# Ascend-Research/HeadPoseEstimation-WHENet

Hardware: AMD Instinct MI355X
Metric: head crops/sec (224x224) (higher is better)
Workload: dtype f16

## Files before the change

### __graft_entry__.py

```python
from __future__ import annotations

import os
import subprocess
import sys
from concurrent.futures import ThreadPoolExecutor

ROOT = os.path.dirname(os.path.abspath(__file__))
PKG = os.path.join(ROOT, "headposeestimation-whenet_amd")
CSRC = os.path.join(PKG, "csrc")
LIBDIR = os.path.join(PKG, "lib")
OBJDIR = os.path.join(PKG, "build")
LIB = os.path.join(LIBDIR, "libwhenet_hip.so")

SOURCES = ["stem.hip", "stemdw.hip", "dw.hip", "se.hip", "pw.hip", "head.hip", "head7.hip", "front.hip", "front2.hip", "front2s.hip", "front7.hip", "mb7.hip", "frame.hip", "headplan.hip", "letterbox.hip", "yolo.hip", "dconv.hip", "convert.hip", "yuv.hip", "ingest.hip", "overlay.hip", "jpeg.hip", "jpeg_dec.hip", "jpeg_dec_seg.hip",
           "snapshot.cpp", "engine.cpp", "engine_post.cpp", "engine_ops.cpp", "detector.cpp", "capi.cpp"]
HEADERS = ["common.h", "spec.h", "snapshot.h", "kernels.h", "device_math.h", "engine.h", "engine_internal.h", "stamps.h", "se_device.h", "overlay_host.h", "jpeg_host.h", "jpeg_dec_host.h", "jpeg_dec_seg_host.h", "front_tuned_f16.inc", "front_tuned_f32.inc", "front2_tuned.inc", "front2s_tuned.inc",
           os.path.join("..", "..", "include", "whenet_hip.h")]
EXTRA_FLAGS = {"front2.hip": ["-mllvm", "-amdgpu-mfma-vgpr-form"], "front2s.hip": ["-mllvm", "-amdgpu-mfma-vgpr-form"], "front7.hip": ["-mllvm", "-amdgpu-mfma-vgpr-form"],
               "mb7.hip": ["-mllvm", "-amdgpu-mfma-vgpr-form"],
               "overlay.hip": ["-ffp-contract=off"]}
CXXFLAGS = ["--offload-arch=gfx950", "-mcode-object-version=5", "-O3", "-std=c++17", "-fPIC", "-Wall",
            "-Wno-unused-function", "-fvisibility=hidden"]


def _hipcc() -> str:
    for cand in (os.environ.get("HIPCC"), "/opt/rocm/bin/hipcc", "hipcc"):
        if cand and (os.path.isabs(cand) and os.path.exists(cand) or not os.path.isabs(cand)):
            return cand
    raise RuntimeError("hipcc not found")


def _stale(target: str, deps) -> bool:
    if not os.path.exists(target):
        return True
    t = os.path.getmtime(target)
    return any(os.path.getmtime(d) > t for d in deps if os.path.exists(d))


def build(force: bool = False, verbose: bool = False) -> None:
    os.makedirs(LIBDIR, exist_ok=True)
    os.makedirs(OBJDIR, exist_ok=True)
    hipcc = _hipcc()
    hdrs = [os.path.join(CSRC, h) for h in HEADERS]

    def compile_one(src: str) -> str:
        s = os.path.join(CSRC, src)
        o = os.path.join(OBJDIR, src.replace(".", "_") + ".o")
        if force or _stale(o, [s] + hdrs):
            cmd = [hipcc] + CXXFLAGS + EXTRA_FLAGS.get(src, []) + ["-c", s, "-o", o]
            if verbose:
                print(" ".join(cmd), flush=True)
            r = subprocess.run(cmd, capture_output=True, text=True)
            if r.returncode != 0:
                raise RuntimeError(f"hipcc failed on {src}:\n{r.stdout}\n{r.stderr}")
        return o

    with ThreadPoolExecutor(max_workers=min(8, len(SOURCES))) as ex:
        objs = list(ex.map(compile_one, SOURCES))
    if force or _stale(LIB, objs):
        cmd = [hipcc, "--offload-arch=gfx950", "-shared", "-fPIC", "-o", LIB] + objs + \
              ["-Wl,-rpath,/opt/rocm/lib", "-Wl,--no-undefined"]
        if verbose:
            print(" ".join(cmd), flush=True)
        r = subprocess.run(cmd, capture_output=True, text=True)
        if r.returncode != 0:
            raise RuntimeError(f"link failed:\n{r.stdout}\n{r.stderr}")
    if PKG not in sys.path:
        sys.path.insert(0, PKG)
    import whenet
    from whenet_hip import _lib
    _lib.load()


def smoke() -> None:
    import numpy as np
    if PKG not in sys.path:
        sys.path.insert(0, PKG)
    if ROOT not in sys.path:
        sys.path.insert(0, ROOT)
    import torch
    from whenet import WHENet
    from whenet_hip import weights as W
    from oracle import whenet_oracle as O

    crops = np.load(os.path.join(ROOT, "tests", "golden", "golden_crops.npy"))[:3]
    w = W.synthetic(1234)
    ref = O.forward(crops, w, np.float64)
    ref_ang = np.stack([ref["yaw"], ref["pitch"], ref["roll"]], axis=1)
    blob = W.pack(w)
    ref_run = np.load(os.path.join(ROOT, "tests", "golden", "reference_get_angle.npz"))["n8_angles"][:3]
    for dtype, tol in (("f32", 1e-3), ("f32s", 1e-3), ("f16", 0.5)):
        m = WHENet(snapshot=blob, dtype=dtype, device=0)
        y, p, r = m.get_angle(crops)
        ang = np.stack([y, p, r], axis=1)
        err = float(np.abs(ang - ref_ang).max())
        err_ref = float(np.abs(ang - ref_run).max())
        print(f"smoke[{dtype}]: max |angle - oracle| = {err:.3e} deg, max |angle - reference-run get_angle| = {err_ref:.3e} deg (tol {tol})")
        assert err <= tol and err_ref <= tol, f"{dtype}: {err} / {err_ref} deg"
        if dtype in ("f32", "f32s"):
            assert np.array_equal(m.last_argmax, ref["argmax"]), "argmax mismatch"
        if dtype == "f32":
            from oracle import preprocess_oracle as P
            from whenet_hip import synth
            from whenet_hip.frames import FramePipeline
            frame, boxes = synth.video_frame(360, 640), synth.head_boxes(3, 360, 640)
            rects_o, crops_o = P.frame_to_crops(frame, boxes)
            with FramePipeline(m) as fp:
                rects, fy, fpi, fr = fp.process(frame, boxes)
            want = m.get_angle(crops_o)
            assert np.array_equal(rects, rects_o) and np.array_equal(fy, want[0]) and np.array_equal(fr, want[2])
            print("smoke[frame]: 3 heads cropped+resized on the device, angles equal to get_angle(oracle crops)")
            import hashlib
            from whenet_hip import yolo
            sample = np.load(os.path.join(ROOT, "tests", "golden", "sample_frames.npz"))["frame0"]
            lb_ref = np.load(os.path.join(ROOT, "tests", "golden", "reference_letterbox.npz"))
            canvas = yolo.letterbox(m, sample, (416, 416), as_uint8=True)
            image_data = yolo.letterbox(m, sample, (416, 416))
            assert hashlib.sha256(canvas.tobytes()).hexdigest() == str(lb_ref["sample0_224x528_to_416x416/sha256"]), "letterbox differs"
            assert image_data.shape == (1, 416, 416, 3) and np.array_equal(image_data[0], canvas.astype(np.float32) / 255)
            print("smoke[letterbox]: 224x528 frame -> 416x416 detector input on the device, equal to the reference's letterbox_image")
            from oracle import yolo_oracle as Y
            maps = synth.yolo_maps(1, num_classes=1)
            kw = dict(max_boxes=20, score_threshold=0.3, iou_threshold=0.45)
            gb, gs, gc, gi, _, _ = m._handle.yolo_eval(maps, synth.YOLO_ANCHORS, 1, (720, 1280), debug=True, **kw)
            rb, rs, rc, ri = Y.yolo_eval(maps, synth.YOLO_ANCHORS, 1, (720, 1280), return_index=True, **kw)
            assert list(gi) == list(ri) and np.allclose(gb, rb, rtol=1e-5, atol=1.0), "yolo_eval differs from the oracle"
            print(f"smoke[yolo]: {len(gb)} detections out of 10647 boxes, same selection as the oracle")
            import json
            from whenet_hip import detector_weights as DW
            with open(os.path.join(ROOT, "tests", "golden", "reference_detector.json")) as f:
                det_meta = json.load(f)
            det_ref = np.load(os.path.join(ROOT, "tests", "golden", "reference_detector.npz"))
            m._handle.detector_load(DW.pack(DW.synthetic(DW.TINY, det_meta["seeds"]["tiny"])))
            det_maps = m._handle.detector_forward(yolo.letterbox(m, sample, (32, 32)), DW.TINY, 18)
            for l, got in enumerate(det_maps):
                want = det_ref[f"tiny/32x32/map{l}"]
                err = float(np.abs(got - want).max() / np.sqrt(np.mean(want ** 2)))
                assert err <= 3 * det_meta["emu_err"]["tiny/32x32"][l], f"detector map {l}: {err}"
            print(f"smoke[detector]: tiny_yolo_body 32x32 on the device, maps {[g.shape[1:3] for g in det_maps]} within the binary16 bound of the executed reference")
            from whenet_hip import _lib
            with open(os.path.join(ROOT, "tests", "golden", "reference_detector_f32.json")) as f:
                e32_body = json.load(f)["e32_body"]["tiny/32x32"]
            h32 = _lib.Handle.postproc(0)
            h32.detector_load(DW.pack(DW.synthetic(DW.TINY, det_meta["seeds"]["tiny"])), dtype="f32")
            for l, got in enumerate(h32.detector_forward(yolo.letterbox(m, sample, (32, 32)), DW.TINY, 18)):
                want = det_ref[f"tiny/32x32/map{l}"]
                err = float(np.abs(got - want).max() / np.sqrt(np.mean(want ** 2)))
                assert err <= 4 * e32_body[l], f"float32 detector map {l}: {err}"
            h32.close()
            print("smoke[detector f32]: the same body with float32 storage, within the float32 bound of the executed reference")
        m.close()
    print("smoke OK")


if __name__ == "__main__":
    build(force="--force" in sys.argv, verbose=True)
    if "--smoke" in sys.argv:
        smoke()
```

### headposeestimation-whenet_amd/csrc/stemdw.hip

```cpp
#include "device_math.h"
#include "kernels.h"
#include "stamps.h"

namespace whenet {

namespace {

constexpr int SD_TH = 16, SD_NSX = 2, SD_TILES_X = 8, SD_TILES_Y = 7;
constexpr int SD_IH = SD_TH + 2, SD_IW = SD_NSX * 7 + 2;
constexpr int SD_NPIX = SD_IH * SD_IW, SD_NSTRIP = SD_NPIX / 32;
constexpr int SD_PR = 2 * SD_IH + 1, SD_PC = 2 * SD_IW + 1;
constexpr int SD_RDW = 26;
constexpr int SD_ROWW = 4 * SD_RDW;
constexpr int SD_C = 32, SD_CG = SD_C / 4, SD_P = 7;
static_assert(SD_NPIX % 32 == 0 && SD_TH * SD_NSX * SD_CG == 256, "tile / lane geometry");

#ifdef WHENET_STEMDW_DEBUG
__device__ half_t* g_stemdw_dbg = nullptr;
#endif

__global__ __launch_bounds__(256) void whenet_stemdw_kernel(const uint8_t* __restrict__ in, half_t* __restrict__ out,
                                                            const StemDwTable* __restrict__ tab, const float* __restrict__ bias,
                                                            const float* __restrict__ wd, const float* __restrict__ bd,
                                                            float* __restrict__ partial) {
    __shared__ uint32_t s_lut[3 * 256];
    __shared__ __attribute__((aligned(16))) uint32_t s_img[SD_PR * SD_ROWW + 8];
    __shared__ __attribute__((aligned(16))) half_t s_tile[SD_NPIX * SD_C];
    __shared__ __attribute__((aligned(16))) float s_w[9 * SD_C];
    float* s_red = reinterpret_cast<float*>(s_tile);

    const int tid = threadIdx.x;
    const int lane = tid & 63, wave = tid >> 6;
    const int g = lane >> 5, lm = lane & 31;
    const int tile = blockIdx.x;
    const int tyi = tile / SD_TILES_X, txi = tile - tyi * SD_TILES_X;
    const int b = blockIdx.y;
    const int oy0 = tyi * SD_TH, ox0 = txi * SD_NSX * SD_P;
    const int sy0 = oy0 - 1, sx0 = ox0 - 1;
    STAMP(0);

    constexpr int NLD = (SD_PR * SD_RDW + 255) / 256;
    const uint8_t* img = in + size_t(b) * IMG * IMG * 3;
    const int byte0 = 6 * sx0 - 2;
    uint32_t raw[NLD];
    bool rok[NLD];
#pragma unroll
    for (int i = 0; i < NLD; ++i) {
        const int d = tid + 256 * i;
        const int r = d / SD_RDW, j = d - r * SD_RDW;
        const int iy = 2 * sy0 + r;
        const int bo = byte0 + 4 * j;
        rok[i] = d < SD_PR * SD_RDW && iy >= 0 && iy < IMG && bo >= 0 && bo < IMG * 3;
        raw[i] = rok[i] ? *reinterpret_cast<const uint32_t*>(img + size_t(iy) * (IMG * 3) + bo) : 0u;
    }
    uint32_t lutv[3];
#pragma unroll
    for (int i = 0; i < 3; ++i) lutv[i] = tab->lut[tid + 256 * i];
    half8 whi[3], wlo[3];
#pragma unroll
    for (int ky = 0; ky < 3; ++ky) {
        whi[ky] = tab->whi[ky][lane];
        wlo[ky] = tab->wlo[ky][lane];
    }
    float4v bv[4];
#pragma unroll
    for (int qq = 0; qq < 4; ++qq) bv[qq] = *reinterpret_cast<const float4v*>(bias + 8 * qq + 4 * g);
    const float wdv0 = wd[tid], wdv1 = (tid < 9 * SD_C - 256) ? wd[256 + tid] : 0.f;
#pragma unroll
    for (int i = 0; i < 3; ++i) s_lut[tid + 256 * i] = lutv[i];
    s_w[tid] = wdv0;
    if (tid < 9 * SD_C - 256) s_w[256 + tid] = wdv1;
    if (tid < 8) s_img[SD_PR * SD_ROWW + tid] = 0u;
    __syncthreads();
    STAMP(1);
#pragma unroll
    for (int i = 0; i < NLD; ++i) {
        const int d = tid + 256 * i;
        if (d >= SD_PR * SD_RDW) continue;
        const int j = d % SD_RDW;
        int ch = (j + 1) % 3;
        uint4 val;
        uint32_t* vp = reinterpret_cast<uint32_t*>(&val);
#pragma unroll
        for (int q = 0; q < 4; ++q) {
            const uint32_t t = s_lut[ch * 256 + ((raw[i] >> (8 * q)) & 0xff)];
            vp[q] = rok[i] ? t : 0u;
            ch = (ch == 2) ? 0 : ch + 1;
        }
        *reinterpret_cast<uint4*>(&s_img[4 * d]) = val;
    }
    __syncthreads();
    STAMP(2);

    for (int strip = wave; strip < SD_NSTRIP; strip += 4) {
        const int p = strip * 32 + lm;
        const int pr = p / SD_IW, pc = p - pr * SD_IW;
        float16v acc;
#pragma unroll
        for (int r = 0; r < 16; ++r) acc[r] = 0.0f;
#pragma unroll
        for (int ky = 0; ky < 3; ++ky) {
            const uint32_t* row = &s_img[(2 * pr + ky) * SD_ROWW + 2 + pc * 6 + 8 * g];
            uint32_t d[8];
#pragma unroll
            for (int i = 0; i < 4; ++i) {
                const uint2 v = *reinterpret_cast<const uint2*>(row + 2 * i);
                d[2 * i] = v.x;
                d[2 * i + 1] = v.y;
            }
            uint32_t ph[4], pl[4];
#pragma unroll
            for (int i = 0; i < 4; ++i) {
                ph[i] = __builtin_amdgcn_perm(d[2 * i + 1], d[2 * i], 0x05040100u);
                pl[i] = __builtin_amdgcn_perm(d[2 * i + 1], d[2 * i], 0x07060302u);
            }
            const half8 xhi = __builtin_bit_cast(half8, uint4{ph[0], ph[1], ph[2], ph[3]});
            const half8 xlo = __builtin_bit_cast(half8, uint4{pl[0], pl[1], pl[2], pl[3]});
            acc = __builtin_amdgcn_mfma_f32_32x32x16_f16(wlo[ky], xhi, acc, 0, 0, 0);
            acc = __builtin_amdgcn_mfma_f32_32x32x16_f16(whi[ky], xlo, acc, 0, 0, 0);
            acc = __builtin_amdgcn_mfma_f32_32x32x16_f16(whi[ky], xhi, acc, 0, 0, 0);
        }
        const int sy = sy0 + pr, sx = sx0 + pc;
        const bool inside = sy >= 0 && sy < STEM_HW && sx >= 0 && sx < STEM_HW;
#pragma unroll
        for (int qq = 0; qq < 4; ++qq) {
            half4 o;
#pragma unroll
            for (int r = 0; r < 4; ++r) o[r] = f32_then_f16(swish_f<false>(acc[4 * qq + r] + bv[qq][r]));
            if (!inside) o = half4{half_t(0.f), half_t(0.f), half_t(0.f), half_t(0.f)};
            *reinterpret_cast<half4*>(s_tile + p * SD_C + 8 * qq + 4 * g) = o;
#ifdef WHENET_STEMDW_DEBUG
            if (inside && g_stemdw_dbg)
                *reinterpret_cast<half4*>(g_stemdw_dbg + ((size_t(b) * STEM_HW + sy) * STEM_HW + sx) * SD_C + 8 * qq + 4 * g) = o;
#endif
        }
    }
    __syncthreads();
    STAMP(3);

    using VCT = half_t __attribute__((ext_vector_type(4)));
    const int cg = tid % SD_CG;
    const int sidx = tid / SD_CG;
    const int ty = sidx / SD_NSX, sx = sidx - ty * SD_NSX;
    const int oy = oy0 + ty;
    float acc[SD_P][4];
#pragma unroll
    for (int p = 0; p < SD_P; ++p)
#pragma unroll
        for (int v = 0; v < 4; ++v) acc[p][v] = 0.0f;
#pragma unroll
    for (int ky = 0; ky < 3; ++ky) {
        float wr[3][4];
#pragma unroll
        for (int kx = 0; kx < 3; ++kx) {
            const float4v t = *reinterpret_cast<const float4v*>(s_w + (ky * 3 + kx) * SD_C + cg * 4);
#pragma unroll
            for (int v = 0; v < 4; ++v) wr[kx][v] = t[v];
        }
        const half_t* row = s_tile + size_t((ty + ky) * SD_IW + sx * SD_P) * SD_C + cg * 4;
#pragma unroll
        for (int ix = 0; ix < SD_P + 2; ++ix) {
            const VCT xv = *reinterpret_cast<const VCT*>(row + ix * SD_C);
            float x[4];
#pragma unroll
            for (int v = 0; v < 4; ++v) x[v] = float(xv[v]);
#pragma unroll
            for (int kx = 0; kx < 3; ++kx) {
                const int d = ix - kx;
                if (d >= 0 && d < SD_P) {
#pragma unroll
                    for (int v = 0; v < 4; ++v) acc[d][v] = fmaf(x[v], wr[kx][v], acc[d][v]);
                }
            }
        }
    }
    STAMP(4);
    float sum[4] = {0.f, 0.f, 0.f, 0.f};
    {
        const float4v bs = *reinterpret_cast<const float4v*>(bd + cg * 4);
        half_t* dst = out + ((size_t(b) * STEM_HW + oy) * STEM_HW + (ox0 + sx * SD_P)) * SD_C + cg * 4;
#pragma unroll
        for (int p = 0; p < SD_P; ++p) {
            VCT o;
#pragma unroll
            for (int v = 0; v < 4; ++v) {
                const float y = opaque_f32(conv_swish<half_t>(acc[p][v] + bs[v]));
                sum[v] += y;
                o[v] = half_t(y);
            }
            *reinterpret_cast<VCT*>(dst + size_t(p) * SD_C) = o;
        }
    }
    STAMP(5);
    lds_barrier();
#pragma unroll
    for (int v = 0; v < 4; ++v) s_red[sidx * SD_C + cg * 4 + v] = sum[v];
    lds_barrier();
    if (tid < SD_C) {
        float t = 0.0f;
        for (int s = 0; s < SD_TH * SD_NSX; ++s) t += s_red[s * SD_C + tid];
        partial[(size_t(b) * (SD_TILES_X * SD_TILES_Y) + tile) * SD_C + tid] = t;
    }
    STAMP(6);
}

__global__ __launch_bounds__(256) void whenet_stemdw_f32_kernel(const uint8_t* __restrict__ in, float* __restrict__ out,
                                                                const float* __restrict__ w, const float* __restrict__ bias,
                                                                const float* __restrict__ lut, const float* __restrict__ wd,
                                                                const float* __restrict__ bd, float* __restrict__ partial) {
    __shared__ __attribute__((aligned(16))) float s_img[SD_PR * SD_ROWW + 8];
    __shared__ __attribute__((aligned(16))) float s_tile[SD_NPIX * SD_C];
    __shared__ __attribute__((aligned(16))) float s_w[9 * SD_C];
    float* s_lut = s_tile;
    float* s_red = s_tile;

    const int tid = threadIdx.x;
    const int lane = tid & 63, wave = tid >> 6;
    const int g = lane >> 5, lm = lane & 31;
    const int tile = blockIdx.x;
    const int tyi = tile / SD_TILES_X, txi = tile - tyi * SD_TILES_X;
    const int b = blockIdx.y;
    const int oy0 = tyi * SD_TH, ox0 = txi * SD_NSX * SD_P;
    const int sy0 = oy0 - 1, sx0 = ox0 - 1;

    constexpr int NLD = (SD_PR * SD_RDW + 255) / 256;
    const uint8_t* img = in + size_t(b) * IMG * IMG * 3;
    const int byte0 = 6 * sx0 - 2;
    uint32_t raw[NLD];
    bool rok[NLD];
#pragma unroll
    for (int i = 0; i < NLD; ++i) {
        const int d = tid + 256 * i;
        const int r = d / SD_RDW, j = d - r * SD_RDW;
        const int iy = 2 * sy0 + r;
        const int bo = byte0 + 4 * j;
        rok[i] = d < SD_PR * SD_RDW && iy >= 0 && iy < IMG && bo >= 0 && bo < IMG * 3;
        raw[i] = rok[i] ? *reinterpret_cast<const uint32_t*>(img + size_t(iy) * (IMG * 3) + bo) : 0u;
    }
    float lutv[3];
#pragma unroll
    for (int i = 0; i < 3; ++i) lutv[i] = lut[tid + 256 * i];
    float wv[3][5];
#pragma unroll
    for (int ky = 0; ky < 3; ++ky)
#pragma unroll
        for (int u = 0; u < 5; ++u) {
            const int j = 2 * u + g;
            wv[ky][u] = (j < 9) ? w[(ky * 9 + j) * STEM_C + lm] : 0.0f;
        }
    float4v bv[4];
#pragma unroll
    for (int qq = 0; qq < 4; ++qq) bv[qq] = *reinterpret_cast<const float4v*>(bias + 8 * qq + 4 * g);
    const float wdv0 = wd[tid], wdv1 = (tid < 9 * SD_C - 256) ? wd[256 + tid] : 0.f;
#pragma unroll
    for (int i = 0; i < 3; ++i) s_lut[tid + 256 * i] = lutv[i];
    s_w[tid] = wdv0;
    if (tid < 9 * SD_C - 256) s_w[256 + tid] = wdv1;
    if (tid < 8) s_img[SD_PR * SD_ROWW + tid] = 0.f;
    __syncthreads();
#pragma unroll
    for (int i = 0; i < NLD; ++i) {
        const int d = tid + 256 * i;
        if (d >= SD_PR * SD_RDW) continue;
        const int j = d % SD_RDW;
        int ch = (j + 1) % 3;
        float4v val;
#pragma unroll
        for (int q = 0; q < 4; ++q) {
            const float t = s_lut[ch * 256 + ((raw[i] >> (8 * q)) & 0xff)];
            val[q] = rok[i] ? t : 0.f;
            ch = (ch == 2) ? 0 : ch + 1;
        }
        *reinterpret_cast<float4v*>(&s_img[4 * d]) = val;
    }
    __syncthreads();

    for (int strip = wave; strip < SD_NSTRIP; strip += 4) {
        const int p = strip * 32 + lm;
        const int pr = p / SD_IW, pc = p - pr * SD_IW;
        float16v acc;
#pragma unroll
        for (int r = 0; r < 16; ++r) acc[r] = 0.0f;
#pragma unroll
        for (int ky = 0; ky < 3; ++ky) {
            const float* row = &s_img[(2 * pr + ky) * SD_ROWW + 2 + pc * 6 + g];
#pragma unroll
            for (int u = 0; u < 5; ++u)
                acc = __builtin_amdgcn_mfma_f32_32x32x2f32(wv[ky][u], row[2 * u], acc, 0, 0, 0);
        }
        const int sy = sy0 + pr, sx = sx0 + pc;
        const bool inside = sy >= 0 && sy < STEM_HW && sx >= 0 && sx < STEM_HW;
#pragma unroll
        for (int qq = 0; qq < 4; ++qq) {
            float4v o;
#pragma unroll
            for (int r = 0; r < 4; ++r) o[r] = opaque_f32(conv_swish<float>(acc[4 * qq + r] + bv[qq][r]));
            if (!inside) o = float4v{0.f, 0.f, 0.f, 0.f};
            *reinterpret_cast<float4v*>(s_tile + p * SD_C + 8 * qq + 4 * g) = o;
        }
    }
    __syncthreads();

    const int cg = tid % SD_CG;
    const int sidx = tid / SD_CG;
    const int ty = sidx / SD_NSX, sx = sidx - ty * SD_NSX;
    const int oy = oy0 + ty;
    float acc[SD_P][4];
#pragma unroll
    for (int p = 0; p < SD_P; ++p)
#pragma unroll
        for (int v = 0; v < 4; ++v) acc[p][v] = 0.0f;
#pragma unroll
    for (int ky = 0; ky < 3; ++ky) {
        float wr[3][4];
#pragma unroll
        for (int kx = 0; kx < 3; ++kx) {
            const float4v t = *reinterpret_cast<const float4v*>(s_w + (ky * 3 + kx) * SD_C + cg * 4);
#pragma unroll
            for (int v = 0; v < 4; ++v) wr[kx][v] = t[v];
        }
        const float* row = s_tile + size_t((ty + ky) * SD_IW + sx * SD_P) * SD_C + cg * 4;
#pragma unroll
        for (int ix = 0; ix < SD_P + 2; ++ix) {
            const float4v xv = *reinterpret_cast<const float4v*>(row + ix * SD_C);
#pragma unroll
            for (int kx = 0; kx < 3; ++kx) {
                const int d = ix - kx;
                if (d >= 0 && d < SD_P) {
#pragma unroll
                    for (int v = 0; v < 4; ++v) acc[d][v] = fmaf(xv[v], wr[kx][v], acc[d][v]);
                }
            }
        }
    }
    float sum[4] = {0.f, 0.f, 0.f, 0.f};
    {
        const float4v bs = *reinterpret_cast<const float4v*>(bd + cg * 4);
        float* dst = out + ((size_t(b) * STEM_HW + oy) * STEM_HW + (ox0 + sx * SD_P)) * SD_C + cg * 4;
#pragma unroll
        for (int p = 0; p < SD_P; ++p) {
            float4v o;
#pragma unroll
            for (int v = 0; v < 4; ++v) {
                const float y = opaque_f32(conv_swish<float>(acc[p][v] + bs[v]));
                sum[v] += y;
                o[v] = y;
            }
            *reinterpret_cast<float4v*>(dst + size_t(p) * SD_C) = o;
        }
    }
    lds_barrier();
#pragma unroll
    for (int v = 0; v < 4; ++v) s_red[sidx * SD_C + cg * 4 + v] = sum[v];
    lds_barrier();
    if (tid < SD_C) {
        float t = 0.0f;
        for (int s = 0; s < SD_TH * SD_NSX; ++s) t += s_red[s * SD_C + tid];
        partial[(size_t(b) * (SD_TILES_X * SD_TILES_Y) + tile) * SD_C + tid] = t;
    }
}

}

bool stemdw_supported(int dtype, const DwPlan& p, int k, int s, int H, int C) {
    const int cv = dtype == WHENET_F16 ? 4 : 8;
    return (dtype == WHENET_F16 || dtype == WHENET_F32) && k == 3 && s == 1 && H == STEM_HW && C == SD_C && p.threads == 256 &&
           p.CV == cv && p.TH == SD_TH && p.NSX == SD_NSX && p.tiles_x == SD_TILES_X && p.tiles_y == SD_TILES_Y && p.chunks == 1;
}

void build_stemdw_table(const float* w, const float* lut, StemDwTable* out) {
    for (int i = 0; i < 3 * 256; ++i) {
        const half_t hi = half_t(lut[i]), lo = half_t(lut[i] - float(hi));
        out->lut[i] = uint32_t(__builtin_bit_cast(unsigned short, hi)) | (uint32_t(__builtin_bit_cast(unsigned short, lo)) << 16);
    }
    for (int ky = 0; ky < 3; ++ky)
        for (int lane = 0; lane < 64; ++lane)
            for (int e = 0; e < 8; ++e) {
                const int j = 8 * (lane >> 5) + e;
                const float v = (j < 9) ? w[(ky * 9 + j) * STEM_C + (lane & 31)] : 0.0f;
                const half_t hi = half_t(v);
                out->whi[ky][lane][e] = hi;
                out->wlo[ky][lane][e] = half_t(v - float(hi));
            }
}

void launch_stemdw(const StemDwArgs& a, hipStream_t stream) {
    WHENET_REQUIRE(a.in && a.out && a.bias && a.wd && a.bd && a.partial && a.n >= 1, WHENET_EINVAL, "stemdw: missing argument");
    if (a.dtype == WHENET_F16) {
        WHENET_REQUIRE(a.tab != nullptr, WHENET_EINVAL, "stemdw: the f16 kernel takes the host-built table");
        hipLaunchKernelGGL(whenet_stemdw_kernel, dim3(SD_TILES_X * SD_TILES_Y, a.n), dim3(256), 0, stream, a.in,
                           static_cast<half_t*>(a.out), a.tab, a.bias, a.wd, a.bd, a.partial);
    } else {
        WHENET_REQUIRE(a.dtype == WHENET_F32 && a.w && a.lut, WHENET_EINVAL, "stemdw: the f32 kernel takes the f32 weights and LUT");
        hipLaunchKernelGGL(whenet_stemdw_f32_kernel, dim3(SD_TILES_X * SD_TILES_Y, a.n), dim3(256), 0, stream, a.in,
                           static_cast<float*>(a.out), a.w, a.bias, a.lut, a.wd, a.bd, a.partial);
    }
    WHENET_HIP_CHECK(hipGetLastError());
}

const char* kernel_name_stemdw(int dtype) { return dtype == WHENET_F16 ? "whenet_stemdw_kernel" : "whenet_stemdw_f32_kernel"; }

}
```

Baseline: 184,500.

## Overlay stem-dw LDS buffers for five workgroups per CU and specialise interior patch loads

The fused stem+depthwise kernel now places the LUT, image patch, output tile, reduction scratch and depthwise weights in one shared byte buffer, with the buffers overlapping. The ninth strip is held in registers by wave 0 until after a barrier, so the weights can be written over the image region first. This keeps LDS use under 32 KB so more workgroups fit on each CU. It also adds templated patch load and LUT conversion paths that drop the bounds checks on interior tiles, uses a fixed five-load lane mapping, and turns on the MFMA VGPR-form compiler flag for this file. In exchange the kernel gains an extra barrier, serialises the last strip onto one wave, and relies on careful aliasing that the static_asserts guard.

```diff
diff --git a/__graft_entry__.py b/__graft_entry__.py
--- a/__graft_entry__.py
+++ b/__graft_entry__.py
@@ -18,6 +18,7 @@
            os.path.join("..", "..", "include", "whenet_hip.h")]
 EXTRA_FLAGS = {"front2.hip": ["-mllvm", "-amdgpu-mfma-vgpr-form"], "front2s.hip": ["-mllvm", "-amdgpu-mfma-vgpr-form"], "front7.hip": ["-mllvm", "-amdgpu-mfma-vgpr-form"],
                "mb7.hip": ["-mllvm", "-amdgpu-mfma-vgpr-form"],
+               "stemdw.hip": ["-mllvm", "-amdgpu-mfma-vgpr-form"],
                "overlay.hip": ["-ffp-contract=off"]}
 CXXFLAGS = ["--offload-arch=gfx950", "-mcode-object-version=5", "-O3", "-std=c++17", "-fPIC", "-Wall",
             "-Wno-unused-function", "-fvisibility=hidden"]
diff --git a/headposeestimation-whenet_amd/csrc/stemdw.hip b/headposeestimation-whenet_amd/csrc/stemdw.hip
--- a/headposeestimation-whenet_amd/csrc/stemdw.hip
+++ b/headposeestimation-whenet_amd/csrc/stemdw.hip
@@ -15,6 +15,49 @@
 constexpr int SD_C = 32, SD_CG = SD_C / 4, SD_P = 7;
 static_assert(SD_NPIX % 32 == 0 && SD_TH * SD_NSX * SD_CG == 256, "tile / lane geometry");
 
+constexpr int SD_SROWS = 9, SD_SDW = SD_SROWS * SD_RDW, SD_NLD = 5;
+static_assert(255 + (SD_NLD - 2) * SD_SDW < SD_PR * SD_RDW && (SD_NLD - 1) * SD_SROWS + 1 == SD_PR,
+              "every lane's four dwords lie in the patch; four slots of nine rows and the last row");
+
+template <bool INTERIOR>
+__device__ __forceinline__ void patch_load(const uint8_t* __restrict__ img, int iy0, int byte0, int tid, uint32_t (&raw)[SD_NLD],
+                                           uint32_t& ok) {
+    const int r0 = tid / SD_RDW, j = tid - r0 * SD_RDW;
+    const int bo = byte0 + 4 * j;
+    const bool colok = INTERIOR || (bo >= 0 && bo < IMG * 3);
+    const uint8_t* src = img + (colok ? bo : 0);
+    ok = 0u;
+#pragma unroll
+    for (int i = 0; i < SD_NLD; ++i) {
+        const int iy = iy0 + (i < SD_NLD - 1 ? r0 + SD_SROWS * i : SD_PR - 1);
+        const bool rowok = INTERIOR || (iy >= 0 && iy < IMG);
+        raw[i] = *reinterpret_cast<const uint32_t*>(src + (rowok ? iy : iy < 0 ? 0 : IMG - 1) * (IMG * 3));
+        ok |= uint32_t(colok && rowok) << i;
+    }
+}
+
+template <bool INTERIOR, typename T>
+__device__ __forceinline__ void patch_to_lds(const T* s_lut, T* s_img, const uint32_t (&raw)[SD_NLD], uint32_t ok, int tid) {
+    using T4 = T __attribute__((ext_vector_type(4)));
+    const int c0 = (tid % SD_RDW + 1) % 3, c1 = (c0 == 2) ? 0 : c0 + 1, c2 = (c1 == 2) ? 0 : c1 + 1;
+    const T* lut[4] = {s_lut + c0 * 256, s_lut + c1 * 256, s_lut + c2 * 256, s_lut + c0 * 256};
+#pragma unroll
+    for (int i = 0; i < SD_NLD; ++i) {
+        if (i == SD_NLD - 1 && tid >= SD_RDW) continue;
+        T4 val;
+#pragma unroll
+        for (int q = 0; q < 4; ++q) {
+            const T t = lut[q][(raw[i] >> (8 * q)) & 0xff];
+            val[q] = (INTERIOR || ((ok >> i) & 1u)) ? t : T(0);
+        }
+        *reinterpret_cast<T4*>(&s_img[4 * (tid + SD_SDW * i)]) = val;
+    }
+}
+
+__device__ __forceinline__ bool patch_interior(int iy0, int byte0) {
+    return iy0 >= 0 && iy0 + SD_PR <= IMG && byte0 >= 0 && byte0 + 4 * SD_RDW <= IMG * 3;
+}
+
 #ifdef WHENET_STEMDW_DEBUG
 __device__ half_t* g_stemdw_dbg = nullptr;
 #endif
@@ -23,11 +66,22 @@
                                                             const StemDwTable* __restrict__ tab, const float* __restrict__ bias,
                                                             const float* __restrict__ wd, const float* __restrict__ bd,
                                                             float* __restrict__ partial) {
-    __shared__ uint32_t s_lut[3 * 256];
-    __shared__ __attribute__((aligned(16))) uint32_t s_img[SD_PR * SD_ROWW + 8];
-    __shared__ __attribute__((aligned(16))) half_t s_tile[SD_NPIX * SD_C];
-    __shared__ __attribute__((aligned(16))) float s_w[9 * SD_C];
-    float* s_red = reinterpret_cast<float*>(s_tile);
+    constexpr int TILE_B = SD_NPIX * SD_C * int(sizeof(half_t)), LAST_B = 32 * SD_C * int(sizeof(half_t));
+    constexpr int IMG_OFF = TILE_B - LAST_B, IMG_B = (SD_PR * SD_ROWW + 8) * 4;
+    constexpr int W_OFF = TILE_B, W_B = 9 * SD_C * 4;
+    constexpr int LDS_B = IMG_OFF + IMG_B;
+    static_assert(LDS_B <= 32768, "five workgroups per CU");
+    static_assert(3 * 256 * 4 <= IMG_OFF && 32 * SD_C * 4 <= TILE_B, "s_lut lies clear of s_img; s_red inside the tile");
+    static_assert(SD_NSTRIP == 9 && 2 * ((SD_NPIX - 32) / SD_IW) == 32, "the ninth strip's first patch row");
+    static_assert(W_OFF == IMG_OFF + LAST_B && W_OFF + W_B - IMG_OFF <= 32 * SD_ROWW * 4,
+                  "what overlies s_img ends in front of patch row 32, and s_w does not touch the ninth strip's pixels");
+    static_assert(IMG_OFF % 16 == 0 && W_OFF % 16 == 0, "vector accesses");
+    __shared__ __attribute__((aligned(16))) unsigned char s_mem[LDS_B];
+    half_t* s_tile = reinterpret_cast<half_t*>(s_mem);
+    uint32_t* s_lut = reinterpret_cast<uint32_t*>(s_mem);
+    uint32_t* s_img = reinterpret_cast<uint32_t*>(s_mem + IMG_OFF);
+    float* s_w = reinterpret_cast<float*>(s_mem + W_OFF);
+    float* s_red = reinterpret_cast<float*>(s_mem);
 
     const int tid = threadIdx.x;
     const int lane = tid & 63, wave = tid >> 6;
@@ -39,20 +93,12 @@
     const int sy0 = oy0 - 1, sx0 = ox0 - 1;
     STAMP(0);
 
-    constexpr int NLD = (SD_PR * SD_RDW + 255) / 256;
     const uint8_t* img = in + size_t(b) * IMG * IMG * 3;
     const int byte0 = 6 * sx0 - 2;
-    uint32_t raw[NLD];
-    bool rok[NLD];
-#pragma unroll
-    for (int i = 0; i < NLD; ++i) {
-        const int d = tid + 256 * i;
-        const int r = d / SD_RDW, j = d - r * SD_RDW;
-        const int iy = 2 * sy0 + r;
-        const int bo = byte0 + 4 * j;
-        rok[i] = d < SD_PR * SD_RDW && iy >= 0 && iy < IMG && bo >= 0 && bo < IMG * 3;
-        raw[i] = rok[i] ? *reinterpret_cast<const uint32_t*>(img + size_t(iy) * (IMG * 3) + bo) : 0u;
-    }
+    const bool interior = patch_interior(2 * sy0, byte0);
+    uint32_t raw[SD_NLD], rok;
+    if (interior) patch_load<true>(img, 2 * sy0, byte0, tid, raw, rok);
+    else patch_load<false>(img, 2 * sy0, byte0, tid, raw, rok);
     uint32_t lutv[3];
 #pragma unroll
     for (int i = 0; i < 3; ++i) lutv[i] = tab->lut[tid + 256 * i];
@@ -68,31 +114,15 @@
     const float wdv0 = wd[tid], wdv1 = (tid < 9 * SD_C - 256) ? wd[256 + tid] : 0.f;
 #pragma unroll
     for (int i = 0; i < 3; ++i) s_lut[tid + 256 * i] = lutv[i];
-    s_w[tid] = wdv0;
-    if (tid < 9 * SD_C - 256) s_w[256 + tid] = wdv1;
     if (tid < 8) s_img[SD_PR * SD_ROWW + tid] = 0u;
     __syncthreads();
     STAMP(1);
-#pragma unroll
-    for (int i = 0; i < NLD; ++i) {
-        const int d = tid + 256 * i;
-        if (d >= SD_PR * SD_RDW) continue;
-        const int j = d % SD_RDW;
-        int ch = (j + 1) % 3;
-        uint4 val;
-        uint32_t* vp = reinterpret_cast<uint32_t*>(&val);
-#pragma unroll
-        for (int q = 0; q < 4; ++q) {
-            const uint32_t t = s_lut[ch * 256 + ((raw[i] >> (8 * q)) & 0xff)];
-            vp[q] = rok[i] ? t : 0u;
-            ch = (ch == 2) ? 0 : ch + 1;
-        }
-        *reinterpret_cast<uint4*>(&s_img[4 * d]) = val;
-    }
+    if (interior) patch_to_lds<true>(s_lut, s_img, raw, rok, tid);
+    else patch_to_lds<false>(s_lut, s_img, raw, rok, tid);
     __syncthreads();
     STAMP(2);
 
-    for (int strip = wave; strip < SD_NSTRIP; strip += 4) {
+    auto stem_strip = [&](int strip, half4 (&o)[4]) {
         const int p = strip * 32 + lm;
         const int pr = p / SD_IW, pc = p - pr * SD_IW;
         float16v acc;
@@ -124,17 +154,33 @@
         const bool inside = sy >= 0 && sy < STEM_HW && sx >= 0 && sx < STEM_HW;
 #pragma unroll
         for (int qq = 0; qq < 4; ++qq) {
-            half4 o;
-#pragma unroll
-            for (int r = 0; r < 4; ++r) o[r] = f32_then_f16(swish_f<false>(acc[4 * qq + r] + bv[qq][r]));
-            if (!inside) o = half4{half_t(0.f), half_t(0.f), half_t(0.f), half_t(0.f)};
-            *reinterpret_cast<half4*>(s_tile + p * SD_C + 8 * qq + 4 * g) = o;
+#pragma unroll
+            for (int r = 0; r < 4; ++r) o[qq][r] = f32_then_f16(swish_f<false>(acc[4 * qq + r] + bv[qq][r]));
+            if (!inside) o[qq] = half4{half_t(0.f), half_t(0.f), half_t(0.f), half_t(0.f)};
+        }
+    };
+    auto store_strip = [&](int strip, const half4 (&o)[4]) {
+        const int p = strip * 32 + lm;
+#pragma unroll
+        for (int qq = 0; qq < 4; ++qq) {
+            *reinterpret_cast<half4*>(s_tile + p * SD_C + 8 * qq + 4 * g) = o[qq];
 #ifdef WHENET_STEMDW_DEBUG
-            if (inside && g_stemdw_dbg)
-                *reinterpret_cast<half4*>(g_stemdw_dbg + ((size_t(b) * STEM_HW + sy) * STEM_HW + sx) * SD_C + 8 * qq + 4 * g) = o;
+            const int sy = sy0 + p / SD_IW, sx = sx0 + p % SD_IW;
+            if (sy >= 0 && sy < STEM_HW && sx >= 0 && sx < STEM_HW && g_stemdw_dbg)
+                *reinterpret_cast<half4*>(g_stemdw_dbg + ((size_t(b) * STEM_HW + sy) * STEM_HW + sx) * SD_C + 8 * qq + 4 * g) = o[qq];
 #endif
         }
-    }
+    };
+    half4 so[4];
+    for (int strip = wave; strip < SD_NSTRIP - 1; strip += 4) {
+        stem_strip(strip, so);
+        store_strip(strip, so);
+    }
+    if (wave == 0) stem_strip(SD_NSTRIP - 1, so);
+    __syncthreads();
+    s_w[tid] = wdv0;
+    if (tid < 9 * SD_C - 256) s_w[256 + tid] = wdv1;
+    if (wave == 0) store_strip(SD_NSTRIP - 1, so);
     __syncthreads();
     STAMP(3);
 
@@ -223,20 +269,12 @@
     const int oy0 = tyi * SD_TH, ox0 = txi * SD_NSX * SD_P;
     const int sy0 = oy0 - 1, sx0 = ox0 - 1;
 
-    constexpr int NLD = (SD_PR * SD_RDW + 255) / 256;
     const uint8_t* img = in + size_t(b) * IMG * IMG * 3;
     const int byte0 = 6 * sx0 - 2;
-    uint32_t raw[NLD];
-    bool rok[NLD];
-#pragma unroll
-    for (int i = 0; i < NLD; ++i) {
-        const int d = tid + 256 * i;
-        const int r = d / SD_RDW, j = d - r * SD_RDW;
-        const int iy = 2 * sy0 + r;
-        const int bo = byte0 + 4 * j;
-        rok[i] = d < SD_PR * SD_RDW && iy >= 0 && iy < IMG && bo >= 0 && bo < IMG * 3;
-        raw[i] = rok[i] ? *reinterpret_cast<const uint32_t*>(img + size_t(iy) * (IMG * 3) + bo) : 0u;
-    }
+    const bool interior = patch_interior(2 * sy0, byte0);
+    uint32_t raw[SD_NLD], rok;
+    if (interior) patch_load<true>(img, 2 * sy0, byte0, tid, raw, rok);
+    else patch_load<false>(img, 2 * sy0, byte0, tid, raw, rok);
     float lutv[3];
 #pragma unroll
     for (int i = 0; i < 3; ++i) lutv[i] = lut[tid + 256 * i];
@@ -258,21 +296,8 @@
     if (tid < 9 * SD_C - 256) s_w[256 + tid] = wdv1;
     if (tid < 8) s_img[SD_PR * SD_ROWW + tid] = 0.f;
     __syncthreads();
-#pragma unroll
-    for (int i = 0; i < NLD; ++i) {
-        const int d = tid + 256 * i;
-        if (d >= SD_PR * SD_RDW) continue;
-        const int j = d % SD_RDW;
-        int ch = (j + 1) % 3;
-        float4v val;
-#pragma unroll
-        for (int q = 0; q < 4; ++q) {
-            const float t = s_lut[ch * 256 + ((raw[i] >> (8 * q)) & 0xff)];
-            val[q] = rok[i] ? t : 0.f;
-            ch = (ch == 2) ? 0 : ch + 1;
-        }
-        *reinterpret_cast<float4v*>(&s_img[4 * d]) = val;
-    }
+    if (interior) patch_to_lds<true>(s_lut, s_img, raw, rok, tid);
+    else patch_to_lds<false>(s_lut, s_img, raw, rok, tid);
     __syncthreads();
 
     for (int strip = wave; strip < SD_NSTRIP; strip += 4) {
```

New measurement: 186,000, median of 6. Within noise of the previous version (+0.8%).
